# warmshao/ChatTTSPlus

Measured on AMD Instinct MI355X. Metric: decode tokens/s, higher is better.
Workload: dtype f32

## Files before the change

chatttsplus_amd/csrc/persist_layer.hip:

```cpp
#include "kernels.h"
#include "persist.h"

typedef unsigned long long u64;

#ifndef PL_LB
#define PL_LB PL_THREADS_MAX
#endif
#define PL_SPIN_LIMIT (1u << 18)

typedef __attribute__((address_space(3))) int pl_lds_int;
#define PL_ABORT_GET(p_) __hip_atomic_load((pl_lds_int*)(p_), __ATOMIC_RELAXED, __HIP_MEMORY_SCOPE_WORKGROUP)
#define PL_ABORT_SET(p_) __hip_atomic_store((pl_lds_int*)(p_), 1, __ATOMIC_RELAXED, __HIP_MEMORY_SCOPE_WORKGROUP)
__device__ inline void store_granule(u64* g, unsigned tag, float v) {
    __hip_atomic_store(g, ((u64)tag << 32) | (u64)__builtin_bit_cast(unsigned, v), __ATOMIC_RELAXED, __HIP_MEMORY_SCOPE_AGENT);
}

template <int N, typename OffFn>
__device__ inline bool sweep(const u64* base, unsigned lane_elem, OffFn off, unsigned tag, float (&v)[N], int* err, int code, int* abort_s, int nap = 1) {
    const u64* p = base + lane_elem;
    asm volatile("" : "+v"(p));
#pragma unroll 1
    for (unsigned spins = 0;; ++spins) {
        bool ok = true;
#pragma unroll
// ... 78 lines not shown
        if (__all(ok)) return true;
        bool giveup = spins >= PL_SPIN_LIMIT || PL_ABORT_GET(abort_s) != 0;
        if (!giveup && (spins & 1023u) == 1023u) giveup = __hip_atomic_load(err, __ATOMIC_RELAXED, __HIP_MEMORY_SCOPE_AGENT) != 0;
        if (giveup) {
            if ((threadIdx.x & 63) == 0) { atomicCAS(err, 0, code); PL_ABORT_SET(abort_s); }
            return false;
        }
        for (int z = 0; z < nap; ++z) __builtin_amdgcn_s_sleep(2);
    }
}
template <int K0, int N, int NE, int TOT>
__device__ __forceinline__ void act16_chunk(const void* g_act, int e, unsigned tag, __attribute__((address_space(3))) float* xs, int* err, int* abort_s, int nap) {
    pl_u32x4 v[N];
    constexpr bool TAIL = (NE * (K0 + N) > TOT);
    const bool got = sweep16<N, TAIL>(g_act, (unsigned)TOT, (unsigned)(e + NE * K0), (unsigned)NE, tag, v, err, 5, abort_s, nap);
    (void)got;
    int ee = e;
    asm volatile("" : "+v"(ee));
#pragma unroll
    for (int k = 0; k < N; ++k) {
        const int f = ee + NE * (K0 + k);
        if (!(TAIL && k == N - 1) || f < TOT) {
            const int P = f / PL_A16_SLOTS, s = f - PL_A16_SLOTS * P;
            __attribute__((address_space(3))) float* const d = xs + 16 * P + 3 * s;
            const unsigned w0 = v[k][0], w1 = v[k][1], w2 = v[k][2];
            d[0] = __builtin_bit_cast(float, w0);
            if (s < 5) { d[1] = __builtin_bit_cast(float, w1); d[2] = __builtin_bit_cast(float, w2); }
        }
    }
}

template <typename OffFn>
__device__ inline void watch_sentinels(const u64* base, OffFn off, int n, unsigned tag, int lane, int* abort_s) {
    const u64* p0 = base + ((lane < n) ? off(lane) : 0);
    const u64* p1 = base + ((lane + 64 < n) ? off(lane + 64) : 0);
    asm volatile("" : "+v"(p0), "+v"(p1));
#pragma unroll 1
    for (unsigned spins = 0; spins < 8192u; ++spins) {
        bool ok = true;
        if (lane < n) ok = (unsigned)(__hip_atomic_load(p0, __ATOMIC_RELAXED, __HIP_MEMORY_SCOPE_AGENT) >> 32) == tag;
        if (lane + 64 < n) ok = ok && ((unsigned)(__hip_atomic_load(p1, __ATOMIC_RELAXED, __HIP_MEMORY_SCOPE_AGENT) >> 32) == tag);
        if (__all(ok) || PL_ABORT_GET(abort_s) != 0) return;
        __builtin_amdgcn_s_sleep(2);
    }
}

template <bool ON> __device__ inline int pl_opq(int idx) {
    if constexpr (ON) asm volatile("" : "+v"(idx));
    return idx;
}
__device__ inline float dot4(const f32x4 w, const f32x4 x, float acc) {
    return fmaf(w[3], x[3], fmaf(w[2], x[2], fmaf(w[1], x[1], fmaf(w[0], x[0], acc))));
}
__device__ inline float dot4(const half4 w, const f32x4 x, float acc) {
    return fmaf((float)w[3], x[3], fmaf((float)w[2], x[2], fmaf((float)w[1], x[1], fmaf((float)w[0], x[0], acc))));
}
template <typename WT> struct PlW;
template <> struct PlW<float> { typedef f32x4 frag; };
template <> struct PlW<half_t> { typedef half4 frag; };
template <typename WT> struct PlKV;
template <> struct PlKV<float> {
    f32x4 a, b;
    __device__ inline void load(const float* p) { a = *(const f32x4*)p; b = *(const f32x4*)(p + 4); }
    __device__ inline float at(int j) const { return j < 4 ? a[j & 3] : b[j & 3]; }
};
template <> struct PlKV<half_t> {
    half8 h;
    __device__ inline void load(const half_t* p) { h = *(const half8*)p; }
    __device__ inline float at(int j) const { return (float)h[j]; }
};
__device__ inline float pl_exp_diff(float m, float mn) { return (m == -INFINITY) ? 0.f : expf(m - mn); }

constexpr int pl_pow2(int n) { return n <= 1 ? 1 : n <= 2 ? 2 : n <= 4 ? 4 : n <= 8 ? 8 : 16; }
template <int CTRL, int C> __device__ inline void pl_rs_step(float* v, bool f) {
    if constexpr (C > 1) {
#pragma unroll
        for (int i = 0; i < C / 2; ++i) {
            const float keep = f ? v[i + C / 2] : v[i];
            const float give = f ? v[i] : v[i + C / 2];
            v[i] = keep + dpp_f<CTRL>(give);
        }
    } else v[0] += dpp_f<CTRL>(v[0]);
}
#define PL_FRONT_BYTES 4096
#ifndef PL_TAIL_ALL
#define PL_TAIL_ALL 1
#endif
#ifndef PL_TAIL_IT
#define PL_TAIL_IT 4
#endif
#define PL_RED_FLOATS (8 * 32 * 4)
template <int P> __device__ inline void pl_reduce_store(float (&v)[P], float* red, int wave, int lane, int base = 0) {
    static_assert(P == 1 || P == 2 || P == 4 || P == 8 || P == 16, "pad to a power of two");
    constexpr int C1 = P > 1 ? P / 2 : 1, C2 = P > 2 ? P / 4 : 1, C3 = P > 4 ? P / 8 : 1;
    const bool f0 = ((lane ^ (lane >> 2)) & 1) != 0, f1 = (((lane >> 1) ^ (lane >> 2)) & 1) != 0, f2 = (((lane >> 2) ^ (lane >> 3)) & 1) != 0, f3 = ((lane >> 3) & 1) != 0;
    pl_rs_step<DPP_XOR1, P>(v, f0);
    pl_rs_step<DPP_XOR2, C1>(v, f1);
    pl_rs_step<DPP_HALF_MIRROR, C2>(v, f2);
    pl_rs_step<DPP_MIRROR, C3>(v, f3);
    int idx = 0;
    bool writer = true;
    if (P > 1) idx += f0 ? P / 2 : 0; else writer = writer && !f0;
    if (C1 > 1) idx += f1 ? C1 / 2 : 0; else writer = writer && !f1;
    if (C2 > 1) idx += f2 ? C2 / 2 : 0; else writer = writer && !f2;
    if (C3 > 1) idx += f3 ? C3 / 2 : 0; else writer = writer && !f3;
    if (writer) red[(wave * 32 + base + idx) * 4 + (lane >> 4)] = v[0];
}
__device__ inline float pl_red(const float* red, int wave, int n) {
    const f32x4 p = *(const f32x4*)(red + (wave * 32 + n) * 4);
    return (p[0] + p[1]) + (p[2] + p[3]);
}
#define PL_PV(N_) float pv[pl_pow2(N_)]; _Pragma("unroll") for (int n_ = 0; n_ < pl_pow2(N_); ++n_) pv[n_] = 0.f

__device__ inline int pl_slot(unsigned long long slots, int r) { return (int)(signed char)(unsigned char)(slots >> (8 * r)); }
template <typename WT> struct PlLoraRegs {
    f32x4 qa_[3], qb_[3], oa_[3], ob_;
    template <typename Q> __device__ inline f32x4& qa(Q&, int j) { return qa_[j]; }
    template <typename Q> __device__ inline f32x4& qb(Q&, int j) { return qb_[j]; }
    template <typename O> __device__ inline f32x4& oa(O&, int j) { return oa_[j]; }
    template <typename Q> __device__ inline f32x4& ob(Q&) { return ob_; }
};
template <> struct PlLoraRegs<float> {
    __device__ inline f32x4& qa(f32x4 (&q_w)[2][3], int j) { return q_w[0][j]; }
    __device__ inline f32x4& qb(f32x4 (&q_w)[2][3], int j) { return q_w[1][j]; }
    __device__ inline f32x4& oa(f32x4 (&o_w)[3], int j) { return o_w[j]; }
    __device__ inline f32x4& ob(f32x4 (&q_w)[2][3]) { return q_w[0][0]; }
};
template <int N>
__device__ inline bool sweep_masked(const u64* base, unsigned lane_elem, bool valid, unsigned tag, float (&v)[N], int* err, int code, int* abort_s, int nap) {
    const u64* p = base + (valid ? lane_elem : 0u);
    asm volatile("" : "+v"(p));
#pragma unroll
    for (int k = 0; k < N; ++k) v[k] = 0.f;
    if (!__any(valid)) return true;
#pragma unroll 1
    for (unsigned spins = 0;; ++spins) {
        bool ok = true;
        if (valid) {
#pragma unroll
            for (int k = 0; k < N; ++k) {
                const u64 x = __hip_atomic_load(p + k, __ATOMIC_RELAXED, __HIP_MEMORY_SCOPE_AGENT);
                v[k] = __builtin_bit_cast(float, (unsigned)x);
                ok = ok && ((unsigned)(x >> 32) == tag);
            }
        }
        if (__all(ok)) return true;
        bool giveup = spins >= PL_SPIN_LIMIT || PL_ABORT_GET(abort_s) != 0;
        if (!giveup && (spins & 1023u) == 1023u) giveup = __hip_atomic_load(err, __ATOMIC_RELAXED, __HIP_MEMORY_SCOPE_AGENT) != 0;
        if (giveup) {
            if ((threadIdx.x & 63) == 0) { atomicCAS(err, 0, code); PL_ABORT_SET(abort_s); }
            return false;
        }
        for (int z = 0; z < nap; ++z) __builtin_amdgcn_s_sleep(2);
    }
}

template <int R, int SCHED, typename WT, bool LORA = false>
__global__ __launch_bounds__(PL_LB) void persist_layer_kernel(const PersistArgs a) {
    static_assert(!LORA || SCHED == 3, "per-utterance adapters: the paced schedule only");
    typedef typename PlW<WT>::frag wfrag;
    constexpr bool A16 = PL_ACT16 != 0 && R <= PL_A16_MAXR;
    constexpr int EW = PL_EDGE_WAVES(R), NE = 64 * EW, GX = 768 / NE;
    constexpr size_t BLOCK_BYTES = (size_t)PL_BLOCK_BYTES / 4 * sizeof(WT), LAYER_BYTES = PL_LAYER_BYTES / 4 * sizeof(WT);
    extern __shared__ __attribute__((aligned(16))) char smem[];
    int* const abort_s = (int*)smem;
    float* const att_s = (float*)(abort_s + 4);
    float* const xs = (float*)(smem + PL_FRONT_BYTES);
    float* const red = xs + R * PL_I;
    float* const ssq = red + PL_RED_FLOATS;
    float* const xres = ssq + 4 * R;
    float* const lbs = xres + 4 * R;
    const int tid = threadIdx.x, lane = tid & 63;
    const int wave = __builtin_amdgcn_readfirstlane(tid >> 6);
    const int b = blockIdx.x;
    const int done_v = vload_flag(a.done), err_v = vload_flag(a.error), ep_v = vload_flag((const int*)a.epoch);
    const int NL = a.n_layers;
    unsigned long long t_mark[10];
#define PL_MARK(i) do { if (a.ts != nullptr) t_mark[i] = wall_clock64(); } while (0)
    PL_MARK(0);
    if (tid == 0) { abort_s[0] = 0; abort_s[1] = 0; }

    if (b < PL_GEMV_BLOCKS) {
        const char* wb = a.w + (size_t)b * BLOCK_BYTES;
        if (wave < 8) {
            const size_t oq = (size_t)wave * (2 * 3 * 64) + lane;
            const size_t oo = (size_t)PL_QKV_BYTES / 16 + (size_t)wave * (3 * 64) + lane;
            const size_t og = (size_t)(PL_QKV_BYTES + PL_O_BYTES) / 16 + (size_t)wave * (4 * 3 * 64) + lane;
            const size_t od = (size_t)(PL_QKV_BYTES + PL_O_BYTES + PL_GU_BYTES) / 16 + (size_t)wave * (6 * 64) + lane;
            wfrag q_w[2][3], o_w[3], g_w[4][3], d_w[6];
#define PL_LOAD_Q(base_) do { if (wave < 6) { _Pragma("unroll") for (int row = 0; row < 2; ++row) _Pragma("unroll") for (int j = 0; j < 3; ++j) \
                q_w[row][j] = __builtin_nontemporal_load((const wfrag*)(base_) + oq + (row * 3 + j) * 64); } } while (0)
#define PL_LOAD_O(base_) do { if (wave < 4) { _Pragma("unroll") for (int j = 0; j < 3; ++j) o_w[j] = __builtin_nontemporal_load((const wfrag*)(base_) + oo + j * 64); } } while (0)
#define PL_LOAD_G(base_) do { _Pragma("unroll") for (int s = 0; s < 4; ++s) _Pragma("unroll") for (int j = 0; j < 3; ++j) \
                g_w[s][j] = __builtin_nontemporal_load((const wfrag*)(base_) + og + (s * 3 + j) * 64); } while (0)
#define PL_LOAD_D(base_) do { _Pragma("unroll") for (int j = 0; j < 6; ++j) d_w[j] = __builtin_nontemporal_load((const wfrag*)(base_) + od + j * 64); } while (0)
            PL_LOAD_Q(wb);
            if (SCHED == 1) PL_LOAD_O(wb);
            PlLoraRegs<WT> lr;
            const unsigned tag0c = (unsigned)ep_v * 32u;
            const int lw = 2 * b + (wave - 6), ll = (wave - 6) * 64 + lane;
            const int lq_r = lw / 48, lq_tk = lw - 48 * lq_r;
            const int lq_sl = (LORA && wave >= 6 && lq_r < R) ? pl_slot(a.lslots, lq_r) : -1;
            const int lo_r = lw >> 4, lo_k = lw & 15;
            const int lo_sl = (LORA && wave >= 6 && lo_r < R) ? pl_slot(a.lslots, lo_r) : -1;
            constexpr int LQM = (192 * R + 127) / 128, LOM = (64 * R + 127) / 128;
#define PL_LORA_REQ_QKV(l_) do { if (wave >= 6) { \
                if (lq_sl >= 0) { const f32x4* ap_ = (const f32x4*)(a.la_qkv + (size_t)(l_) * a.la_qkv_stride + (size_t)(lq_sl * 48 + lq_tk) * PL_H); \
                    _Pragma("unroll") for (int j = 0; j < 3; ++j) lr.qa(q_w, j) = ap_[64 * j + lane]; \
                    lq_scale = a.lscale[((l_) * 8 + lq_sl) * 4 + (lq_tk >> 4)]; } \
                int li_ = ll; asm volatile("" : "+v"(li_)); \
                _Pragma("unroll") for (int m = 0; m < LQM; ++m) { const int i_ = li_ + 128 * m; float v_ = 0.f; \
                    if (i_ < 192 * R) { const int r_ = i_ / 192, rem_ = i_ - 192 * r_, j_ = rem_ >> 4, k_ = rem_ & 15, sl_ = pl_slot(a.lslots, r_); \
                        if (sl_ >= 0) { const int pw_ = j_ >> 1, hf_ = j_ & 1, hh_ = b >> 4, jj_ = b & 15; \
                            const int t_ = pw_ < 4 ? (pw_ >> 1) : 2, d_ = pw_ < 4 ? 2 * jj_ + (pw_ & 1) + 32 * hf_ : 4 * jj_ + 2 * (pw_ - 4) + hf_; \
                            v_ = a.lb[(size_t)(l_) * a.la_stride + (size_t)((sl_ * 4 + t_) * 16 + k_) * PL_H + hh_ * 64 + d_]; } } \
                    lr.qb(q_w, m >> 2)[m & 3] = v_; } } } while (0)
#define PL_LORA_REQ_O(l_) do { if (wave >= 6) { \
                if (lo_sl >= 0) { const f32x4* ap_ = (const f32x4*)(a.la + (size_t)(l_) * a.la_stride + (size_t)((lo_sl * 4 + 3) * 16 + lo_k) * PL_H); \
                    _Pragma("unroll") for (int j = 0; j < 3; ++j) lr.oa(o_w, j) = ap_[64 * j + lane]; \
                    lo_scale = a.lscale[((l_) * 8 + lo_sl) * 4 + 3]; } \
                int li_ = ll; asm volatile("" : "+v"(li_)); \
                _Pragma("unroll") for (int m = 0; m < LOM; ++m) { const int i_ = li_ + 128 * m; float v_ = 0.f; \
                    if (i_ < 64 * R) { const int r_ = i_ >> 6, ii_ = (i_ >> 4) & 3, k_ = i_ & 15, sl_ = pl_slot(a.lslots, r_); \
                        if (sl_ >= 0) v_ = a.lb[(size_t)(l_) * a.la_stride + (size_t)((sl_ * 4 + 3) * 16 + k_) * PL_H + 4 * b + ii_]; } \
                    lr.ob(q_w)[m] = v_; } } } while (0)
            float lq_scale = 0.f, lo_scale = 0.f;
            if constexpr (LORA) PL_LORA_REQ_QKV(0);
            __builtin_amdgcn_sched_barrier(0);
            if (__builtin_amdgcn_readfirstlane(done_v | err_v)) return;
            __syncthreads();
            if constexpr (SCHED == 3) {
                typedef __attribute__((address_space(3))) int lds_int;
                lds_int* const arrive = (lds_int*)(abort_s + 1);
                int phase = 0;
                const int pace = a.pace;
#define PL_PACE_BEGIN() const int tgt_ = EW * (++phase); bool ready_ = __hip_atomic_load(arrive, __ATOMIC_RELAXED, __HIP_MEMORY_SCOPE_WORKGROUP) >= tgt_
#define PL_PIECE(stmt_) do { stmt_; if (!ready_) { for (int z_ = 0; z_ < pace; ++z_) __builtin_amdgcn_s_sleep(2); ready_ = __hip_atomic_load(arrive, __ATOMIC_RELAXED, __HIP_MEMORY_SCOPE_WORKGROUP) >= tgt_; } } while (0)
#define PL_PACE_END() do { while (!ready_) { __builtin_amdgcn_s_sleep(1); ready_ = __hip_atomic_load(arrive, __ATOMIC_RELAXED, __HIP_MEMORY_SCOPE_WORKGROUP) >= tgt_; } asm volatile("" ::: "memory"); } while (0)
                for (int l = 0; l < NL; ++l) {
                    const char* const wn = wb + LAYER_BYTES;
                    const bool more = l + 1 < NL;
                    {
                        PL_PACE_BEGIN();
                        if (wave < 4) {
#pragma unroll
                            for (int j = 0; j < 3; ++j) PL_PIECE(o_w[j] = __builtin_nontemporal_load((const wfrag*)wb + oo + j * 64));
                        }
                        PL_PACE_END();
                    }
                    if constexpr (LORA) if (wave >= 6) {
                        if (lq_sl >= 0) {
                            float acc = 0.f;
#pragma unroll
                            for (int j = 0; j < 3; ++j) acc = dot4(lr.qa(q_w, j), ((const f32x4*)(xs + lq_r * PL_H))[64 * j + lane], acc);
                            acc = wave_sum(acc);
                            const float rs = 1.0f / sqrtf((EW == 2 ? ssq[lq_r] + ssq[R + lq_r] : (ssq[lq_r] + ssq[R + lq_r]) + (ssq[2 * R + lq_r] + ssq[3 * R + lq_r])) / (float)PL_H + a.eps);
                            if (lane == 0) store_granule(a.g_u + lq_r * 64 + lq_tk, tag0c + (unsigned)l, (acc * rs) * lq_scale);
                        }
#pragma unroll
                        for (int m = 0; m < LQM; ++m) if (ll + 128 * m < 192 * R) lbs[ll + 128 * m] = lr.qb(q_w, m >> 2)[m & 3];
                    }
                    if (wave < 6) {
                        PL_PV(2 * R);
#pragma unroll
                        for (int r = 0; r < R; ++r) {
                            f32x4 xr[3];
#pragma unroll
                            for (int j = 0; j < 3; ++j) xr[j] = ((const f32x4*)(xs + r * PL_H))[64 * j + lane];
#pragma unroll
                            for (int row = 0; row < 2; ++row) {
                                float acc = 0.f;
#pragma unroll
                                for (int j = 0; j < 3; ++j) acc = dot4(q_w[row][j], xr[j], acc);
                                pv[row * R + r] = acc;
                            }
                        }
                        pl_reduce_store<pl_pow2(2 * R)>(pv, red, wave, lane);
                    }
                    __syncthreads();
                    if constexpr (LORA) PL_LORA_REQ_O(l);
                    {
                        PL_PACE_BEGIN();
#pragma unroll
                        for (int s = 0; s < 4; ++s)
#pragma unroll
                            for (int j = 0; j < 3; ++j) PL_PIECE(g_w[s][j] = __builtin_nontemporal_load((const wfrag*)wb + og + (s * 3 + j) * 64));
                        PL_PACE_END();
                    }
                    if constexpr (LORA) if (wave >= 6) {
                        if (lo_sl >= 0) {
                            float acc = 0.f;
#pragma unroll
                            for (int j = 0; j < 3; ++j) acc = dot4(lr.oa(o_w, j), ((const f32x4*)(xs + lo_r * PL_H))[64 * j + lane], acc);
                            acc = wave_sum(acc);
                            if (lane == 0) store_granule(a.g_u + lo_r * 64 + 48 + lo_k, tag0c + (unsigned)l, acc * lo_scale);
                        }
#pragma unroll
                        for (int m = 0; m < LOM; ++m) if (ll + 128 * m < 64 * R) lbs[192 * R + ll + 128 * m] = lr.ob(q_w)[m];
                    }
                    if (wave < 4) {
                        PL_PV(R);
#pragma unroll
                        for (int r = 0; r < R; ++r) {
                            float acc = 0.f;
#pragma unroll
                            for (int j = 0; j < 3; ++j) acc = dot4(o_w[j], ((const f32x4*)(xs + r * PL_H))[64 * j + lane], acc);
                            pv[r] = acc;
                        }
                        pl_reduce_store<pl_pow2(R)>(pv, red, wave, lane);
                    }
                    __syncthreads();
                    {
                        PL_PACE_BEGIN();
#pragma unroll
                        for (int j = 0; j < 6; ++j) PL_PIECE(d_w[j] = __builtin_nontemporal_load((const wfrag*)wb + od + j * 64));
                        PL_PACE_END();
                    }
#ifdef PL_EXP_E2
                    if constexpr (R == 5) {
#else
                    if constexpr (R >= 5) {
// ... 116 lines not shown
#pragma unroll
                    for (int j = 0; j < 3; ++j) xr[r][j] = ((const f32x4*)(xs + r * PL_H))[64 * j + lane];
                if (wave < 6) {
                    PL_PV(2 * R);
#pragma unroll
                    for (int row = 0; row < 2; ++row)
#pragma unroll
                        for (int r = 0; r < R; ++r) {
                            float acc = 0.f;
#pragma unroll
                            for (int j = 0; j < 3; ++j) acc = dot4(q_w[row][j], xr[r][j], acc);
                            pv[row * R + r] = acc;
                        }
                    pl_reduce_store<pl_pow2(2 * R)>(pv, red, wave, lane);
                }
                if (SCHED == 2) PL_LOAD_O(wb);
                PL_LOAD_G(wb);
                if (SCHED == 1 && more) PL_LOAD_Q(wn);
                __builtin_amdgcn_sched_barrier(0);
                __syncthreads();
                __syncthreads();
#pragma unroll
                for (int r = 0; r < R; ++r)
#pragma unroll
                    for (int j = 0; j < 3; ++j) xr[r][j] = ((const f32x4*)(xs + r * PL_H))[64 * j + lane];
                if (wave < 4) {
                    PL_PV(R);
#pragma unroll
                    for (int r = 0; r < R; ++r) {
                        float acc = 0.f;
#pragma unroll
                        for (int j = 0; j < 3; ++j) acc = dot4(o_w[j], xr[r][j], acc);
                        pv[r] = acc;
                    }
                    pl_reduce_store<pl_pow2(R)>(pv, red, wave, lane);
                }
                PL_LOAD_D(wb);
                if (SCHED == 1 && more) PL_LOAD_O(wn);
                __builtin_amdgcn_sched_barrier(0);
                __syncthreads();
                __syncthreads();
#pragma unroll
                for (int r = 0; r < R; ++r)
#pragma unroll
                    for (int j = 0; j < 3; ++j) xr[r][j] = ((const f32x4*)(xs + r * PL_H))[64 * j + lane];
                {
                    float pv[2][pl_pow2(2 * R)];
#pragma unroll
                    for (int n = 0; n < pl_pow2(2 * R); ++n) { pv[0][n] = 0.f; pv[1][n] = 0.f; }
#pragma unroll
                    for (int s = 0; s < 4; ++s)
#pragma unroll
                        for (int r = 0; r < R; ++r) {
                            float acc = 0.f;
#pragma unroll
                            for (int j = 0; j < 3; ++j) acc = dot4(g_w[s][j], xr[r][j], acc);
                            pv[s >> 1][(s & 1) * R + r] = acc;
                        }
                    pl_reduce_store<pl_pow2(2 * R)>(pv[0], red, wave, lane, 0);
                    pl_reduce_store<pl_pow2(2 * R)>(pv[1], red, wave, lane, 16);
                }
                __builtin_amdgcn_sched_barrier(0);
                __syncthreads();
                __syncthreads();
                const int half = wave & 1;
                {
                    PL_PV(R);
#pragma unroll
                    for (int r = 0; r < R; ++r) {
                        float acc = 0.f;
#pragma unroll
                        for (int j = 0; j < 6; ++j) acc = dot4(d_w[j], ((const f32x4*)(xs + r * PL_I))[384 * half + 64 * j + lane], acc);
                        pv[r] = acc;
                    }
                    pl_reduce_store<pl_pow2(R)>(pv, red, wave, lane);
                }
                if (SCHED == 2 && more) PL_LOAD_Q(wn);
                __builtin_amdgcn_sched_barrier(0);
                __syncthreads();
                wb = wn;
            }
        } else {
#define PL_B1() do { if (SCHED == 3) { asm volatile("s_waitcnt lgkmcnt(0)" ::: "memory"); \
        if (lane == 0) __hip_atomic_fetch_add((__attribute__((address_space(3))) int*)(abort_s + 1), 1, __ATOMIC_RELAXED, __HIP_MEMORY_SCOPE_WORKGROUP); } \
        else __syncthreads(); } while (0)

            const int ew = wave - 8, e = ew * 64 + lane;
            const int hh = b >> 4, jj = b & 15;
            const int tA = e, pwA = tA % 6, rA = (tA / 6 < R) ? tA / 6 : 0;
            const bool doA = tA < 6 * R;
            RowMeta mA = {0, 0, 0, 0};
            float cA = 1.f, sA = 0.f;
            if (doA) {
                mA = a.meta[rA];
                if (pwA < 4) {
                    const int d = 2 * jj + (pwA & 1);
                    cA = a.rope_rows[(size_t)rA * 64 + d];
                    sA = a.rope_rows[(size_t)rA * 64 + 32 + d];
                }
            }
            constexpr int XIT = (R * 192 + NE - 1) / NE;
            f32x4 xv[XIT];
#pragma unroll
            for (int i = 0; i < XIT; ++i) {
                const int idx = e + NE * i;
                xv[i] = (idx < R * 192) ? ((const f32x4*)a.x)[idx] : (f32x4){0.f, 0.f, 0.f, 0.f};
            }
            f32x4 xown = {0.f, 0.f, 0.f, 0.f};
            if (e < R) xown = *(const f32x4*)(a.x + (size_t)e * PL_H + 4 * b);
            if (__builtin_amdgcn_readfirstlane(done_v | err_v)) return;
            const unsigned tag0 = (unsigned)ep_v * 32u;
            if (e < R) *(f32x4*)(xres + 4 * e) = xown;
            float ssp[R];
#pragma unroll
            for (int r = 0; r < R; ++r) ssp[r] = 0.f;
#pragma unroll
            for (int i = 0; i < XIT; ++i) {
                const int idx = e + NE * i;
                if (idx < R * 192) ((f32x4*)xs)[idx] = xv[i];
                const float d = xv[i][0] * xv[i][0] + xv[i][1] * xv[i][1] + xv[i][2] * xv[i][2] + xv[i][3] * xv[i][3];
#pragma unroll
                for (int r = 0; r < R; ++r) ssp[r] += (idx / 192 == r) ? d : 0.f;
            }
#pragma unroll
            for (int r = 0; r < R; ++r) {
                const float s = wave_sum(ssp[r]);
                if (lane == 0) ssq[ew * R + r] = s;
            }
            __syncthreads();
            PL_MARK(1);
            const size_t kv_per = a.kv_per;
            for (int l = 0; l < NL; ++l) {
                const unsigned tag = tag0 + (unsigned)l;
                const bool last = l + 1 == NL;
                if (l > 0) {
                    for (int z = 0; z < a.delay_x; ++z) __builtin_amdgcn_s_sleep(2);
                    if (EW == 2 && (a.poll & 1)) watch_sentinels(a.g_x, [ew](int i) { return (R - 1) * PL_H + 4 * (16 * (2 * (i >> 4) + ew) + (i & 15)) + 3; }, 96, tag - 1u, lane, abort_s);
                    float v[GX * R];
                    const bool got = PL_SWEEP(GX * R, a.g_x, PL_G_X, (unsigned)e, [](int k) { return (k / GX) * PL_H + NE * (k % GX); }, tag - 1u, v, 1);
                    (void)got;
#pragma unroll
                    for (int r = 0; r < R; ++r) ssp[r] = 0.f;
#pragma unroll
                    for (int k = 0; k < GX * R; ++k) {
                        xs[(k / GX) * PL_H + NE * (k % GX) + e] = v[k];
                        ssp[k / GX] += v[k] * v[k];
                    }
#pragma unroll
                    for (int r = 0; r < R; ++r) {
                        const float s = wave_sum(ssp[r]);
                        if (lane == 0) ssq[ew * R + r] = s;
                    }
                }
                if (last) PL_MARK(2);
                PL_B1();
                float lda = 0.f, ldb = 0.f;
                float uq[LORA ? 16 : 1];
                const int slA = (LORA && doA) ? pl_slot(a.lslots, rA) : -1;
                if constexpr (LORA) {
                    for (int z = 0; z < a.delay_u; ++z) __builtin_amdgcn_s_sleep(2);
                    const bool got = sweep_masked<16>(a.g_u, (unsigned)(rA * 64 + (pwA < 4 ? (pwA >> 1) : 2) * 16), slA >= 0, tag, uq, a.error, 9, abort_s, a.nap);
                    (void)got;
                }
                __syncthreads();
                if constexpr (LORA) {
                    if (slA >= 0) {
                        const float* const bq = lbs + rA * 192 + 2 * pwA * 16;
#pragma unroll
                        for (int k = 0; k < 16; ++k) { lda = fmaf(bq[k], uq[k], lda); ldb = fmaf(bq[16 + k], uq[k], ldb); }
                    }
                }
                if (doA) {
                    const float rs = 1.0f / sqrtf((EW == 2 ? ssq[rA] + ssq[R + rA] : (ssq[rA] + ssq[R + rA]) + (ssq[2 * R + rA] + ssq[3 * R + rA])) / (float)PL_H + a.eps);
                    const float va = pl_red(red, pwA, rA) * rs + lda, vb = pl_red(red, pwA, R + rA) * rs + ldb;
                    float ya = va, yb = vb;
                    int which, dA, dB;
                    if (pwA < 4) {
                        which = pwA >> 1; dA = 2 * jj + (pwA & 1); dB = dA + 32;
                        ya = __fadd_rn(__fmul_rn(va, cA), __fmul_rn(-vb, sA));
                        yb = __fadd_rn(__fmul_rn(vb, cA), __fmul_rn(va, sA));
                    } else {
                        which = 2; dA = 4 * jj + 2 * (pwA - 4); dB = dA + 1;
                    }
                    u64* const gq = a.g_qkv + (size_t)pl_opq<(R > PL_MAXR_ONE)>((rA * PL_NH + hh) * 192 + which * 64);
                    store_granule(gq + dA, tag, ya);
                    store_granule(gq + dB, tag, yb);
                    if (which >= 1) {
                        WT* c = (WT*)a.kv + (size_t)l * 2 * kv_per + (which == 2 ? kv_per : 0) + (((size_t)mA.seq * PL_NH + hh) * a.Lmax + mA.slot) * CTTS_HEAD_DIM;
                        c[dA] = (WT)ya; c[dB] = (WT)yb;
                    }
                }
                if (last) PL_MARK(3);
                for (int z = 0; z < a.delay_att; ++z) __builtin_amdgcn_s_sleep(2);
                {
                    if (EW == 2 && (a.poll & 1)) watch_sentinels(a.g_att, [ew](int i) { return (i / 6) * PL_H + 64 * (2 * (i % 6) + ew) + 63; }, 6 * R, tag, lane, abort_s);
                    float v[GX * R];
                    const bool got = PL_SWEEP(GX * R, a.g_att, PL_G_ATT, (unsigned)e, [](int k) { return (k / GX) * PL_H + NE * (k % GX); }, tag, v, 3);
                    (void)got;
#pragma unroll
                    for (int k = 0; k < GX * R; ++k) xs[(k / GX) * PL_H + NE * (k % GX) + e] = v[k];
                }
                if (last) PL_MARK(4);
                PL_B1();
                float ldo = 0.f;
                float uo[LORA ? 16 : 1];
                const int slO = (LORA && e < 4 * R) ? pl_slot(a.lslots, e >> 2) : -1;
                if constexpr (LORA) {
                    for (int z = 0; z < a.delay_u; ++z) __builtin_amdgcn_s_sleep(2);
                    const bool got = sweep_masked<16>(a.g_u, (unsigned)((e >> 2) * 64 + 48), slO >= 0, tag, uo, a.error, 10, abort_s, a.nap);
                    (void)got;
                }
                __syncthreads();
                if constexpr (LORA) {
                    if (slO >= 0) {
                        const float* const bo = lbs + 192 * R + (e >> 2) * 64 + (e & 3) * 16;
#pragma unroll
                        for (int k = 0; k < 16; ++k) ldo = fmaf(bo[k], uo[k], ldo);
                    }
                }
                if (e < 4 * R) {
                    const int i = e & 3, r = e >> 2;
                    const float x1 = xres[4 * r + i] + (pl_red(red, i, r) + ldo);
                    xres[4 * r + i] = x1;
                    if (!(a.fault > 0 && b == 5 && l + 1 == a.fault))
                        store_granule(a.g_x1 + (size_t)pl_opq<(R > PL_MAXR_ONE)>(r * PL_H + 4 * b + i), tag, x1);
                }
                if (last) PL_MARK(5);
                for (int z = 0; z < a.delay; ++z) __builtin_amdgcn_s_sleep(2);
                {
                    if (EW == 2 && (a.poll & 1)) watch_sentinels(a.g_x1, [ew](int i) { return (R - 1) * PL_H + 4 * (16 * (2 * (i >> 4) + ew) + (i & 15)) + 3; }, 96, tag, lane, abort_s);
                    float v[GX * R];
                    const bool got = PL_SWEEP(GX * R, a.g_x1, PL_G_X1, (unsigned)e, [](int k) { return (k / GX) * PL_H + NE * (k % GX); }, tag, v, 4);
                    (void)got;
#pragma unroll
                    for (int r = 0; r < R; ++r) ssp[r] = 0.f;
#pragma unroll
                    for (int k = 0; k < GX * R; ++k) {
                        xs[(k / GX) * PL_H + NE * (k % GX) + e] = v[k];
                        ssp[k / GX] += v[k] * v[k];
                    }
#pragma unroll
                    for (int r = 0; r < R; ++r) {
                        const float s = wave_sum(ssp[r]);
                        if (lane == 0) ssq[ew * R + r] = s;
                    }
                }
                if (last) PL_MARK(6);
                PL_B1();
                __syncthreads();
                if constexpr (A16) {
                    float av = 0.f;
                    const int pi = e & 15, r = e >> 4;
                    if (e < 16 * R) {
                        const int w = pi >> 1, p = pi & 1;
                        const float rs = 1.0f / sqrtf((EW == 2 ? ssq[r] + ssq[R + r] : (ssq[r] + ssq[R + r]) + (ssq[2 * R + r] + ssq[3 * R + r])) / (float)PL_H + a.eps);
                        const float gv = pl_red(red, w, 16 * p + r) * rs, uv = pl_red(red, w, 16 * p + R + r) * rs;
                        av = (gv / (1.0f + expf(-gv))) * uv;
                    }
                    const float a1 = __shfl_down(av, 1), a2 = __shfl_down(av, 2);
                    if (e < 16 * R && pi % 3 == 0)
                        store_granule16(a.g_act, PL_GEMV_BLOCKS * PL_A16_SLOTS * R, (unsigned)pl_opq<(R > PL_MAXR_ONE)>((r * PL_GEMV_BLOCKS + b) * PL_A16_SLOTS + pi / 3), tag,
                                        av, (pi + 1 < 16) ? a1 : 0.f, (pi + 2 < 16) ? a2 : 0.f);
                } else if (e < 16 * R) {
                    const int pi = e & 15, r = e >> 4, w = pi >> 1, p = pi & 1;
                    const float rs = 1.0f / sqrtf((EW == 2 ? ssq[r] + ssq[R + r] : (ssq[r] + ssq[R + r]) + (ssq[2 * R + r] + ssq[3 * R + r])) / (float)PL_H + a.eps);
                    const float gv = pl_red(red, w, 16 * p + r) * rs, uv = pl_red(red, w, 16 * p + R + r) * rs;
                    store_granule(a.g_act + (size_t)pl_opq<(R > PL_MAXR_ONE)>(r * PL_I + 16 * b + pi), tag, (gv / (1.0f + expf(-gv))) * uv);
                }
                if (last) PL_MARK(7);
                for (int z = 0; z < a.delay_act; ++z) __builtin_amdgcn_s_sleep(2);
                if constexpr (A16) {
                    constexpr int TOT = PL_GEMV_BLOCKS * PL_A16_SLOTS * R, NK = (TOT + NE - 1) / NE;
                    constexpr int NC = (NK + PL_A16_CHUNK - 1) / PL_A16_CHUNK, CH = (NK + NC - 1) / NC;
                    act16_chunk<0, (NK < CH ? NK : CH), NE, TOT>(a.g_act, e, tag, (__attribute__((address_space(3))) float*)xs, a.error, abort_s, a.nap);
                    if constexpr (NC > 1) act16_chunk<CH, (NK - CH < CH ? NK - CH : CH), NE, TOT>(a.g_act, e, tag, (__attribute__((address_space(3))) float*)xs, a.error, abort_s, a.nap);
                    if constexpr (NC > 2) act16_chunk<2 * CH, (NK - 2 * CH < CH ? NK - 2 * CH : CH), NE, TOT>(a.g_act, e, tag, (__attribute__((address_space(3))) float*)xs, a.error, abort_s, a.nap);
                    if constexpr (NC > 3) act16_chunk<3 * CH, (NK - 3 * CH < CH ? NK - 3 * CH : CH), NE, TOT>(a.g_act, e, tag, (__attribute__((address_space(3))) float*)xs, a.error, abort_s, a.nap);
                    if constexpr (NC > 4) act16_chunk<4 * CH, NK - 4 * CH, NE, TOT>(a.g_act, e, tag, (__attribute__((address_space(3))) float*)xs, a.error, abort_s, a.nap);
                    static_assert(NC <= 5, "act gather: more chunks");
                } else {
                if (EW == 2 && (a.poll & 1)) watch_sentinels(a.g_act, [ew](int i) { return (R - 1) * PL_I + 16 * (8 * (i >> 2) + 4 * ew + (i & 3)) + 15; }, 96, tag, lane, abort_s);
                if constexpr (EW == 2) {
#pragma unroll
                    for (int r = 0; r < R; ++r) {
                        float v[24];
                        const bool got = sweep<24>(a.g_act, (unsigned)(r * PL_I + e), [](int k) { return 128 * k; }, tag, v, a.error, 5, abort_s, a.nap);
                        (void)got;
#pragma unroll
                        for (int k = 0; k < 24; ++k) xs[r * PL_I + 128 * k + e] = v[k];
                    }
                } else {
#ifdef PL_EXP_E1
                    if constexpr (R > PL_MAXR_ONE) {
#pragma unroll
                        for (int r = 0; r < R; ++r) {
                            float v[12];
                            const bool got = PL_SWEEP(12, a.g_act, PL_G_ACT, (unsigned)(r * PL_I + e), [](int k) { return 256 * k; }, tag, v, 5);
                            (void)got;
#pragma unroll
                            for (int k = 0; k < 12; ++k) xs[r * PL_I + 256 * k + e] = v[k];
                        }
                    } else
#endif
#pragma unroll
                    for (int r = 0; r + 1 < R; r += 2) {
                        float v[24];
                        const bool got = PL_SWEEP(24, a.g_act, PL_G_ACT, (unsigned)(r * PL_I + e), [](int k) { return (k / 12) * PL_I + 256 * (k % 12); }, tag, v, 5);
                        (void)got;
#pragma unroll
                        for (int k = 0; k < 24; ++k) xs[(r + k / 12) * PL_I + 256 * (k % 12) + e] = v[k];
                    }
#ifdef PL_EXP_E1
                    if constexpr ((R & 1) != 0 && R <= PL_MAXR_ONE) {
#else
                    if constexpr ((R & 1) != 0) {
#endif
                        constexpr int r = R - 1;
                        float v[12];
                        const bool got = PL_SWEEP(12, a.g_act, PL_G_ACT, (unsigned)(r * PL_I + e), [](int k) { return 256 * k; }, tag, v, 5);
                        (void)got;
#pragma unroll
                        for (int k = 0; k < 12; ++k) xs[r * PL_I + 256 * k + e] = v[k];
                    }
                }
                }
                if (last) PL_MARK(8);
                PL_B1();
                __syncthreads();
                if (e < 4 * R) {
                    const int i = e & 3, r = e >> 2;
                    const float x2 = xres[4 * r + i] + (pl_red(red, 2 * i, r) + pl_red(red, 2 * i + 1, r));
                    if (last && !a.heads) a.x[(size_t)r * PL_H + 4 * b + i] = x2;
                    else {
                        xres[4 * r + i] = x2;
                        store_granule(a.g_x + (size_t)pl_opq<(R > PL_MAXR_ONE)>(r * PL_H + 4 * b + i), tag, x2);
                    }
                }
            }
            if (a.heads) {
                const unsigned tagh = tag0 + (unsigned)(NL - 1);
                int4 hst = make_int4(1, 0, 0, 0);
                int hout = 0;
                float lnf_v = 0.f;
                if (e < 4 * R) {
                    hst = *(const int4*)(a.rows + (e >> 2));
                    hout = a.rows[e >> 2].out;
                    lnf_v = a.lnf[4 * b + (e & 3)];
                }
                for (int z = 0; z < a.delay_x; ++z) __builtin_amdgcn_s_sleep(2);
                float v[GX * R];
                const bool got = PL_SWEEP(GX * R, a.g_x, PL_G_X, (unsigned)e, [](int k) { return (k / GX) * PL_H + NE * (k % GX); }, tagh, v, 1);
                (void)got;
#pragma unroll
                for (int r = 0; r < R; ++r) ssp[r] = 0.f;
#pragma unroll
                for (int k = 0; k < GX * R; ++k) {
                    xs[(k / GX) * PL_H + NE * (k % GX) + e] = v[k];
                    ssp[k / GX] += v[k] * v[k];
                }
#pragma unroll
                for (int r = 0; r < R; ++r) {
                    const float s = wave_sum(ssp[r]);
                    if (lane == 0) ssq[ew * R + r] = s;
                }
                PL_B1();
                __syncthreads();
                if (e < PL_HEAD_ROWS * R) {
                    const int rr = e % PL_HEAD_ROWS, r = e / PL_HEAD_ROWS, col = PL_HEAD_ROWS * b + rr;
                    const float rs = 1.0f / sqrtf((EW == 2 ? ssq[r] + ssq[R + r] : (ssq[r] + ssq[R + r]) + (ssq[2 * R + r] + ssq[3 * R + r])) / (float)PL_H + a.eps);
                    if (col < a.n_valid) a.logits[(size_t)r * a.n_valid + col] = pl_red(red, rr >> 1, (rr & 1) * R + r) * rs;
                }
                if (e < 4 * R) {
                    float* const hid_out = ((SamplerDynPtr)a.dyn)->hidden_out;
                    if (hid_out != nullptr && hst.x == 0) {
                        const int i = e & 3, r = e >> 2;
                        const float rs = 1.0f / sqrtf((EW == 2 ? ssq[r] + ssq[R + r] : (ssq[r] + ssq[R + r]) + (ssq[2 * R + r] + ssq[3 * R + r])) / (float)PL_H + a.eps);
                        hid_out[(size_t)hout * ((SamplerDynPtr)a.dyn)->hidden_stride + (size_t)hst.y * PL_H + 4 * b + i] = lnf_v * (xres[4 * r + i] * rs);
                    }
                }
            }
            PL_MARK(9);
            if (a.ts != nullptr && e == 0) {
#pragma unroll
                for (int i = 0; i < 10; ++i) a.ts[(size_t)b * 10 + i] = t_mark[i];
            }
            if (b == 0 && e == 0) __hip_atomic_fetch_add(a.epoch, 1u, __ATOMIC_RELAXED, __HIP_MEMORY_SCOPE_AGENT);
        }
        return;
    }

    constexpr bool PAIR = R > PL_MAXR_ONE;
    constexpr int NWI = PAIR ? 4 : 8;
    const int S = PAIR ? 1 : a.S;
    const int isub = PAIR ? ((wave < 8) ? (wave >> 2) : ((wave - 8) & 1)) : 0;
    const int iw = PAIR ? (wave & 3) : wave;
    const int item = PAIR ? 2 * (b - PL_GEMV_BLOCKS) + isub : b - PL_GEMV_BLOCKS;
    if ((PAIR ? 2 * (b - PL_GEMV_BLOCKS) : item) >= PL_NH * R * S) return;
    const int rh = item / S, sp = item - rh * S;
    const int r = rh / PL_NH, hh = rh % PL_NH;
    float* const qs = att_s + 64 * isub;
    float* const ks = att_s + 128 + 64 * isub;
    float* const vs = att_s + 256 + 64 * isub;
    float* const mo = att_s + 384;
    float* const mm = mo + 512;
    float* const ml = mm + 8;
    const size_t kv_per = a.kv_per;
    if (wave < 8) {
        const RowMeta m = a.meta[r];
        const int kvc = (m.slot - m.kv_start + S - 1) / S;
        const int kv0 = m.kv_start + sp * kvc, kv1 = min(kv0 + kvc, m.slot);
        const int grp = lane >> 3, sub = lane & 7;
        const size_t head_base = ((size_t)m.seq * PL_NH + hh) * a.Lmax * CTTS_HEAD_DIM;
        constexpr int PRE = 6;
        constexpr int NT = (PAIR || PL_TAIL_ALL) ? PL_TAIL_IT : 0, PT = PRE + NT;
        constexpr int TB = sizeof(WT) == 4 ? 4096 : 2048;
        typedef __attribute__((address_space(3))) char lds_c;
        typedef __attribute__((address_space(1))) const void* gptr_t;
        lds_c* const tl = (lds_c*)smem + PL_FRONT_BYTES + wave * (NT * TB);
        PlKV<WT> kf[PRE];
        typename KvElem<WT>::reg vv[PRE][8];
        bool ok[PT];
        bool any_ok[PT];
#pragma unroll
        for (int u = 0; u < PT; ++u) {
            const int p = kv0 + 8 * (iw + NWI * u) + grp;
            ok[u] = p < kv1;
            any_ok[u] = kv0 + 8 * (iw + NWI * u) < kv1;
        }
#define PL_LOAD_KV(l_) do { const WT* const kb_ = (const WT*)a.kv + (size_t)(l_) * 2 * kv_per + head_base; const WT* const vb_ = kb_ + kv_per + lane; \
        _Pragma("unroll") for (int u = 0; u < PRE; ++u) if (any_ok[u]) { const int p0_ = kv0 + 8 * (iw + NWI * u); const int pc_ = ok[u] ? p0_ + grp : m.kv_start; \
            kf[u].load(kb_ + (size_t)pc_ * CTTS_HEAD_DIM + 8 * sub); \
            _Pragma("unroll") for (int g = 0; g < 8; ++g) vv[u][g] = KvElem<WT>::load(vb_ + (size_t)min(p0_ + g, kv1 - 1) * CTTS_HEAD_DIM); } } while (0)
#define PL_DMA_KV(l_) do { if constexpr (NT > 0) { const WT* const kb_ = (const WT*)a.kv + (size_t)(l_) * 2 * kv_per + head_base; const WT* const vb_ = kb_ + kv_per; \
        int ln_ = lane; asm volatile("" : "+v"(ln_));       \
        const int grp = ln_ >> 3, sub = ln_ & 7, lane = ln_; \
        _Pragma("unroll") for (int t = 0; t < NT; ++t) if (any_ok[PRE + t]) { const int p0_ = kv0 + 8 * (iw + NWI * (PRE + t)); \
            const WT* const ks_ = kb_ + (size_t)min(p0_ + grp, kv1 - 1) * CTTS_HEAD_DIM + 8 * sub; \
            if constexpr (sizeof(WT) == 4) { \
                __builtin_amdgcn_global_load_lds((gptr_t)ks_, (__attribute__((address_space(3))) void*)(tl + t * TB), 16, 0, 0); \
                __builtin_amdgcn_global_load_lds((gptr_t)(ks_ + 4), (__attribute__((address_space(3))) void*)(tl + t * TB + 1024), 16, 0, 0); \
                const WT* const v0_ = vb_ + (size_t)min(p0_ + (lane >> 4), kv1 - 1) * CTTS_HEAD_DIM + 4 * (lane & 15); \
                const WT* const v1_ = vb_ + (size_t)min(p0_ + 4 + (lane >> 4), kv1 - 1) * CTTS_HEAD_DIM + 4 * (lane & 15); \
                __builtin_amdgcn_global_load_lds((gptr_t)v0_, (__attribute__((address_space(3))) void*)(tl + t * TB + 2048), 16, 0, 0); \
                __builtin_amdgcn_global_load_lds((gptr_t)v1_, (__attribute__((address_space(3))) void*)(tl + t * TB + 3072), 16, 0, 0); \
            } else { \
                __builtin_amdgcn_global_load_lds((gptr_t)ks_, (__attribute__((address_space(3))) void*)(tl + t * TB), 16, 0, 0); \
                const WT* const v0_ = vb_ + (size_t)min(p0_ + grp, kv1 - 1) * CTTS_HEAD_DIM + 8 * sub; \
                __builtin_amdgcn_global_load_lds((gptr_t)v0_, (__attribute__((address_space(3))) void*)(tl + t * TB + 1024), 16, 0, 0); \
            } } } } while (0)
        PL_DMA_KV(0);
        PL_LOAD_KV(0);
        __builtin_amdgcn_sched_barrier(0);
// ... 328 lines not shown
```

Measured before the change: 3898.

## Arrive before sum-of-squares reduction, use hardware barrier wake, DPP shifts for act16

Edge waves now signal arrival to the GEMV waves before computing and storing the RMS-norm sum-of-squares, so the paced GEMV phase can start earlier. The GEMV waves' paced spin-wait and the edge arrival are replaced by an s_barrier pairing, which wakes waiting waves directly instead of polling with sleeps. Cross-lane shuffles in the act16 packing are swapped for DPP row shifts. An optional early per-row rsqrt path with its own LDS counter is added but stays disabled by default. The barrier pairing requires both wave groups to execute matching s_barrier counts, which risks deadlock if the counts ever diverge.

```diff
diff --git a/chatttsplus_amd/csrc/persist_layer.hip b/chatttsplus_amd/csrc/persist_layer.hip
--- a/chatttsplus_amd/csrc/persist_layer.hip
+++ b/chatttsplus_amd/csrc/persist_layer.hip
@@ -184,6 +184,24 @@
         }
     } else v[0] += dpp_f<CTRL>(v[0]);
 }
+#ifndef PL_EARLY_ARRIVE
+#define PL_EARLY_ARRIVE 1
+#endif
+#ifndef PL_RS_EARLY
+#define PL_RS_EARLY 0
+#endif
+#ifndef PL_TRIM_NORM_MAXR
+#define PL_TRIM_NORM_MAXR 1
+#endif
+#ifndef PL_BAR_WAKE
+#define PL_BAR_WAKE 1
+#endif
+#ifndef PL_A16_DPP
+#define PL_A16_DPP 1
+#endif
+#define PL_DPP_ROW_SHL(n_) (0x100 + (n_))
+__device__ inline float pl_row_shl1(float v) { return __builtin_bit_cast(float, __builtin_amdgcn_update_dpp(0, __builtin_bit_cast(int, v), PL_DPP_ROW_SHL(1), 0xF, 0xF, true)); }
+__device__ inline float pl_row_shl2(float v) { return __builtin_bit_cast(float, __builtin_amdgcn_update_dpp(0, __builtin_bit_cast(int, v), PL_DPP_ROW_SHL(2), 0xF, 0xF, true)); }
 #define PL_FRONT_BYTES 4096
 #ifndef PL_TAIL_ALL
 #define PL_TAIL_ALL 1
@@ -260,6 +278,9 @@
 template <int R, int SCHED, typename WT, bool LORA = false>
 __global__ __launch_bounds__(PL_LB) void persist_layer_kernel(const PersistArgs a) {
     static_assert(!LORA || SCHED == 3, "per-utterance adapters: the paced schedule only");
+    constexpr bool EARLY = PL_EARLY_ARRIVE != 0 && SCHED == 3 && !LORA && R <= PL_TRIM_NORM_MAXR;
+    constexpr bool RSE = PL_RS_EARLY != 0 && SCHED == 3 && !LORA && R <= PL_TRIM_NORM_MAXR;
+    constexpr bool BARW = PL_BAR_WAKE != 0 && SCHED == 3;
     typedef typename PlW<WT>::frag wfrag;
     constexpr bool A16 = PL_ACT16 != 0 && R <= PL_A16_MAXR;
     constexpr int EW = PL_EDGE_WAVES(R), NE = 64 * EW, GX = 768 / NE;
@@ -280,7 +301,7 @@
     unsigned long long t_mark[10];
 #define PL_MARK(i) do { if (a.ts != nullptr) t_mark[i] = wall_clock64(); } while (0)
     PL_MARK(0);
-    if (tid == 0) { abort_s[0] = 0; abort_s[1] = 0; }
+    if (tid == 0) { abort_s[0] = 0; abort_s[1] = 0; abort_s[2] = 0; }
 
     if (b < PL_GEMV_BLOCKS) {
         const char* wb = a.w + (size_t)b * BLOCK_BYTES;
@@ -338,7 +359,8 @@
                 const int pace = a.pace;
 #define PL_PACE_BEGIN() const int tgt_ = EW * (++phase); bool ready_ = __hip_atomic_load(arrive, __ATOMIC_RELAXED, __HIP_MEMORY_SCOPE_WORKGROUP) >= tgt_
 #define PL_PIECE(stmt_) do { stmt_; if (!ready_) { for (int z_ = 0; z_ < pace; ++z_) __builtin_amdgcn_s_sleep(2); ready_ = __hip_atomic_load(arrive, __ATOMIC_RELAXED, __HIP_MEMORY_SCOPE_WORKGROUP) >= tgt_; } } while (0)
-#define PL_PACE_END() do { while (!ready_) { __builtin_amdgcn_s_sleep(1); ready_ = __hip_atomic_load(arrive, __ATOMIC_RELAXED, __HIP_MEMORY_SCOPE_WORKGROUP) >= tgt_; } asm volatile("" ::: "memory"); } while (0)
+#define PL_PACE_END() do { if constexpr (BARW) { (void)ready_; asm volatile("s_waitcnt lgkmcnt(0)\n\ts_barrier" ::: "memory"); } \
+        else { while (!ready_) { __builtin_amdgcn_s_sleep(1); ready_ = __hip_atomic_load(arrive, __ATOMIC_RELAXED, __HIP_MEMORY_SCOPE_WORKGROUP) >= tgt_; } asm volatile("" ::: "memory"); } } while (0)
                 for (int l = 0; l < NL; ++l) {
                     const char* const wn = wb + LAYER_BYTES;
                     const bool more = l + 1 < NL;
@@ -621,8 +643,19 @@
             }
         } else {
 #define PL_B1() do { if (SCHED == 3) { asm volatile("s_waitcnt lgkmcnt(0)" ::: "memory"); \
-        if (lane == 0) __hip_atomic_fetch_add((__attribute__((address_space(3))) int*)(abort_s + 1), 1, __ATOMIC_RELAXED, __HIP_MEMORY_SCOPE_WORKGROUP); } \
+        if (lane == 0) __hip_atomic_fetch_add((__attribute__((address_space(3))) int*)(abort_s + 1), 1, __ATOMIC_RELAXED, __HIP_MEMORY_SCOPE_WORKGROUP); \
+        if constexpr (BARW) asm volatile("s_barrier" ::: "memory"); } \
         else __syncthreads(); } while (0)
+            typedef __attribute__((address_space(3))) int pl_lds_cnt;
+#define PL_SSQ_COUNT() do { if constexpr (RSE) { asm volatile("s_waitcnt lgkmcnt(0)" ::: "memory"); \
+        if (lane == 0) __hip_atomic_fetch_add((pl_lds_cnt*)(abort_s + 2), 1, __ATOMIC_RELAXED, __HIP_MEMORY_SCOPE_WORKGROUP); } } while (0)
+#define PL_SSQ_STORE() do { _Pragma("unroll") for (int r = 0; r < R; ++r) { const float s_ = wave_sum(ssp[r]); if (lane == 0) ssq[ew * R + r] = s_; } PL_SSQ_COUNT(); } while (0)
+#define PL_SSQ_WAIT(code_, norms_) do { const int t2_ = EW * (norms_);       \
+        for (unsigned sp_ = 0; __hip_atomic_load((pl_lds_cnt*)(abort_s + 2), __ATOMIC_RELAXED, __HIP_MEMORY_SCOPE_WORKGROUP) < t2_; ++sp_) { \
+            if (sp_ >= PL_SPIN_LIMIT || PL_ABORT_GET(abort_s) != 0) { if (lane == 0) { atomicCAS(a.error, 0, code_); PL_ABORT_SET(abort_s); } break; } \
+            __builtin_amdgcn_s_sleep(1); } \
+        asm volatile("" ::: "memory"); } while (0)
+#define PL_RS(r_) (1.0f / sqrtf((EW == 2 ? ssq[r_] + ssq[R + (r_)] : (ssq[r_] + ssq[R + (r_)]) + (ssq[2 * R + (r_)] + ssq[3 * R + (r_)])) / (float)PL_H + a.eps))
 
             const int ew = wave - 8, e = ew * 64 + lane;
             const int hh = b >> 4, jj = b & 15;
@@ -661,12 +694,15 @@
 #pragma unroll
                 for (int r = 0; r < R; ++r) ssp[r] += (idx / 192 == r) ? d : 0.f;
             }
-#pragma unroll
-            for (int r = 0; r < R; ++r) {
-                const float s = wave_sum(ssp[r]);
-                if (lane == 0) ssq[ew * R + r] = s;
+            if constexpr (!EARLY) {
+#pragma unroll
+                for (int r = 0; r < R; ++r) {
+                    const float s = wave_sum(ssp[r]);
+                    if (lane == 0) ssq[ew * R + r] = s;
+                }
             }
             __syncthreads();
+            if constexpr (!EARLY) PL_SSQ_COUNT();
             PL_MARK(1);
             const size_t kv_per = a.kv_per;
             for (int l = 0; l < NL; ++l) {
@@ -685,14 +721,25 @@
                         xs[(k / GX) * PL_H + NE * (k % GX) + e] = v[k];
                         ssp[k / GX] += v[k] * v[k];
                     }
-#pragma unroll
-                    for (int r = 0; r < R; ++r) {
-                        const float s = wave_sum(ssp[r]);
-                        if (lane == 0) ssq[ew * R + r] = s;
-                    }
-                }
-                if (last) PL_MARK(2);
-                PL_B1();
+                    if constexpr (EARLY) {
+                        if (last) PL_MARK(2);
+                        PL_B1();
+                    }
+                    PL_SSQ_STORE();
+                } else if constexpr (EARLY) {
+                    if (last) PL_MARK(2);
+                    PL_B1();
+                    PL_SSQ_STORE();
+                }
+                if constexpr (!EARLY) {
+                    if (last) PL_MARK(2);
+                    PL_B1();
+                }
+                float rsA = 0.f;
+                if constexpr (RSE) if (ew * 64 < 6 * R) {
+                    PL_SSQ_WAIT(1, 2 * l + 1);
+                    if (doA) rsA = PL_RS(rA);
+                }
                 float lda = 0.f, ldb = 0.f;
                 float uq[LORA ? 16 : 1];
                 const int slA = (LORA && doA) ? pl_slot(a.lslots, rA) : -1;
@@ -710,7 +757,7 @@
                     }
                 }
                 if (doA) {
-                    const float rs = 1.0f / sqrtf((EW == 2 ? ssq[rA] + ssq[R + rA] : (ssq[rA] + ssq[R + rA]) + (ssq[2 * R + rA] + ssq[3 * R + rA])) / (float)PL_H + a.eps);
+                    const float rs = RSE ? rsA : PL_RS(rA);
                     const float va = pl_red(red, pwA, rA) * rs + lda, vb = pl_red(red, pwA, R + rA) * rs + ldb;
                     float ya = va, yb = vb;
                     int which, dA, dB;
@@ -778,31 +825,38 @@
                         xs[(k / GX) * PL_H + NE * (k % GX) + e] = v[k];
                         ssp[k / GX] += v[k] * v[k];
                     }
-#pragma unroll
-                    for (int r = 0; r < R; ++r) {
-                        const float s = wave_sum(ssp[r]);
-                        if (lane == 0) ssq[ew * R + r] = s;
-                    }
-                }
-                if (last) PL_MARK(6);
-                PL_B1();
+                    if constexpr (EARLY) {
+                        if (last) PL_MARK(6);
+                        PL_B1();
+                    }
+                    PL_SSQ_STORE();
+                }
+                if constexpr (!EARLY) {
+                    if (last) PL_MARK(6);
+                    PL_B1();
+                }
+                float rsD = 0.f;
+                if constexpr (RSE) if (ew * 64 < 16 * R) {
+                    PL_SSQ_WAIT(4, 2 * l + 2);
+                    if (e < 16 * R) rsD = PL_RS(e >> 4);
+                }
                 __syncthreads();
                 if constexpr (A16) {
                     float av = 0.f;
                     const int pi = e & 15, r = e >> 4;
                     if (e < 16 * R) {
                         const int w = pi >> 1, p = pi & 1;
-                        const float rs = 1.0f / sqrtf((EW == 2 ? ssq[r] + ssq[R + r] : (ssq[r] + ssq[R + r]) + (ssq[2 * R + r] + ssq[3 * R + r])) / (float)PL_H + a.eps);
+                        const float rs = RSE ? rsD : PL_RS(r);
                         const float gv = pl_red(red, w, 16 * p + r) * rs, uv = pl_red(red, w, 16 * p + R + r) * rs;
                         av = (gv / (1.0f + expf(-gv))) * uv;
                     }
-                    const float a1 = __shfl_down(av, 1), a2 = __shfl_down(av, 2);
+                    const float a1 = PL_A16_DPP ? pl_row_shl1(av) : __shfl_down(av, 1), a2 = PL_A16_DPP ? pl_row_shl2(av) : __shfl_down(av, 2);
                     if (e < 16 * R && pi % 3 == 0)
                         store_granule16(a.g_act, PL_GEMV_BLOCKS * PL_A16_SLOTS * R, (unsigned)pl_opq<(R > PL_MAXR_ONE)>((r * PL_GEMV_BLOCKS + b) * PL_A16_SLOTS + pi / 3), tag,
                                         av, (pi + 1 < 16) ? a1 : 0.f, (pi + 2 < 16) ? a2 : 0.f);
                 } else if (e < 16 * R) {
                     const int pi = e & 15, r = e >> 4, w = pi >> 1, p = pi & 1;
-                    const float rs = 1.0f / sqrtf((EW == 2 ? ssq[r] + ssq[R + r] : (ssq[r] + ssq[R + r]) + (ssq[2 * R + r] + ssq[3 * R + r])) / (float)PL_H + a.eps);
+                    const float rs = RSE ? rsD : PL_RS(r);
                     const float gv = pl_red(red, w, 16 * p + r) * rs, uv = pl_red(red, w, 16 * p + R + r) * rs;
                     store_granule(a.g_act + (size_t)pl_opq<(R > PL_MAXR_ONE)>(r * PL_I + 16 * b + pi), tag, (gv / (1.0f + expf(-gv))) * uv);
                 }
@@ -897,16 +951,18 @@
                     xs[(k / GX) * PL_H + NE * (k % GX) + e] = v[k];
                     ssp[k / GX] += v[k] * v[k];
                 }
-#pragma unroll
-                for (int r = 0; r < R; ++r) {
-                    const float s = wave_sum(ssp[r]);
-                    if (lane == 0) ssq[ew * R + r] = s;
-                }
-                PL_B1();
+                if constexpr (EARLY) PL_B1();
+                PL_SSQ_STORE();
+                if constexpr (!EARLY) PL_B1();
+                float rsH = 0.f;
+                if constexpr (RSE) if (ew * 64 < PL_HEAD_ROWS * R) {
+                    PL_SSQ_WAIT(1, 2 * NL + 1);
+                    if (e < PL_HEAD_ROWS * R) rsH = PL_RS(e / PL_HEAD_ROWS);
+                }
                 __syncthreads();
                 if (e < PL_HEAD_ROWS * R) {
                     const int rr = e % PL_HEAD_ROWS, r = e / PL_HEAD_ROWS, col = PL_HEAD_ROWS * b + rr;
-                    const float rs = 1.0f / sqrtf((EW == 2 ? ssq[r] + ssq[R + r] : (ssq[r] + ssq[R + r]) + (ssq[2 * R + r] + ssq[3 * R + r])) / (float)PL_H + a.eps);
+                    const float rs = RSE ? rsH : PL_RS(r);
                     if (col < a.n_valid) a.logits[(size_t)r * a.n_valid + col] = pl_red(red, rr >> 1, (rr & 1) * R + r) * rs;
                 }
                 if (e < 4 * R) {
```

After: 4040 (median of 6 runs). 3.7% higher.
